# schusto/k-means-demo

Hardware: AMD Instinct MI355X
Metric: Lloyd iterations/sec (and point-assignments/sec) at N=1e8, D=128, K=1024, 1/2/4/8 MI355X (higher is better)
Workload: dtype bf16; 1 GPU; model=kmeans-lloyd N=1e8 D=128 K=1024, global_batch=100000000, seq_len=128, n_points=100000000, n_features=128, n_clusters=1024, parallelism=dp1

## Files before the change

### mikmeans/csrc/assign16.hip

```cpp
#include <cstdlib>
#include <type_traits>

#include "common.h"
#include "kernels.h"
#include "plan.h"
#include "tile.h"

namespace mk {

using plan::chunk_tiles16;

template <typename T, int DPAD, int P_, int CT_ = 0, int NBUF_ = 2, int NW_ = 4>
struct Assign16Cfg {
  static constexpr int NW = NW_;
  static constexpr int P = P_;
  static constexpr int V = Elem<T>::V;
  static constexpr int NQ = DPAD / 4 / V;
  static constexpr int TILE_BYTES = NQ * 1024;
  static constexpr int CT = CT_ ? CT_ : chunk_tiles16(sizeof(T), DPAD);
  static constexpr int CHUNK_BYTES = CT * TILE_BYTES;
  static constexpr int PIECES = CHUNK_BYTES / 1024;
  static constexpr int NPW = PIECES / NW;
  static constexpr int PTS = NW * P * 16;
  static constexpr int PP = (P + 3) / 4 * 4;
// ... 618 lines not shown
      blds16(rC, (MK_LDS void*)(dst + pc * 1024), loff, src + (uint32_t)pc * 1024u);
    }
  };
  const int64_t N = a.N;
  float* red = (float*)(bufs + C::NBUF * C::CHUNK_BYTES);
  float* opt = (float*)(bufs + C::NBUF * C::CHUNK_BYTES + 16 * C::NW);
  double* wacc = (double*)(bufs + C::NBUF * C::CHUNK_BYTES + 16 * C::NW + C::OPT_BYTES);
  uint32_t* xg_lds = (uint32_t*)(opt + C::NW * 16 * C::PP);
  uint32_t* el_lds = (uint32_t*)(bufs + C::NBUF * C::CHUNK_BYTES + 16 * C::NW + C::OPT_BYTES + 16 * C::NW);
  const unsigned kmask = key6_mask();
  const int G = (int)gridDim.x;
  int grp = (int)blockIdx.x;
  unsigned* ctr = g_persist_ctr[cslot];
  int* nxt_lds = (int*)(red + 2 * C::NW);
  int s0 = 0;

  const uint32_t rowb = (uint32_t)a.ldx * (uint32_t)sizeof(T);
  auto rows_of = [&](int gi) -> int {
    const int64_t left = N - (int64_t)gi * C::PTS;
    return left < C::PTS ? (int)left : C::PTS;
  };
  auto fresh_tid = []() -> int {
    int t = (int)threadIdx.x;
    asm volatile("" : "+v"(t));
    return t;
  };
  auto sx = [](int ln, int v, int o) -> int { return __builtin_amdgcn_ds_bpermute((ln ^ o) << 2, v); };
  auto sxf = [&](int ln, float v, int o) -> float { return __int_as_float(sx(ln, __float_as_int(v), o)); };
  auto lrow_of = [&](int tid, int p) -> int { return wid * (C::P * 16) + p * 16 + (tid & 15); };

// ... 30 lines not shown
  };

  if (a.timeline && threadIdx.x == 0) {
    const unsigned long long t = __builtin_amdgcn_s_memrealtime();
    a.timeline[(int64_t)grp * 8] = t;
    a.timeline[(int64_t)grp * 8 + 7] = t;
  }
  auto issue_cn = [&]() {
    const __amdgpu_buffer_rsrc_t rN = make_rsrc(a.cn, (uint32_t)a.Kpad * 4u);
    for (int pc = wid; pc < cn_bytes / 1024; pc += C::NW)
      blds16(rN, (MK_LDS void*)(cn_lds + pc * 1024), loff, (uint32_t)pc * 1024u);
  };
  issue_cn();
  issue_chunk(0, 0);
  load_group(grp);
  for (;;) {
    const int nvc = rows_of(grp);
    int nxt = 0;
    bool has_next = false;
    wait_vmcnt<0>();
    if (a.timeline && threadIdx.x == 0) a.timeline[(int64_t)grp * 8 + 6] = __builtin_amdgcn_s_memrealtime();
    float exn[EJ];
    exn[0] = __uint_as_float(xg_lds[fresh_tid()]);
    float off = 0.f;
    bool ppo = false;
    unsigned fetched;
    {
      const int ttid = fresh_tid();
      fetched = 0u;
      const int tln = ttid & 63, tr = ttid & 15, tg = tln >> 4;
      float m = 0.f, mn = 3.0e38f;
#pragma unroll
      for (int j = 0; j < EJ; ++j) { m = fmaxf(m, exn[j]); mn = fminf(mn, exn[j]); }
      m = fmaxf(m, sxf(tln, m, 16));
      mn = fminf(mn, sxf(tln, mn, 16));
      m = fmaxf(m, sxf(tln, m, 32));
      mn = fminf(mn, sxf(tln, mn, 32));
#pragma unroll
      for (int o = 1; o < 16; o <<= 1) {
        m = fmaxf(m, sxf(tln, m, o));
        mn = fminf(mn, sxf(tln, mn, o));
      }
      if (tln == 0) { red[2 * wid] = m; red[2 * wid + 1] = mn; }
      wait_lgkm0();
      raw_barrier();
      float mnw = 3.0e38f;
#pragma unroll
      for (int w = 0; w < C::NW; ++w) { off = fmaxf(off, red[2 * w]); mnw = fminf(mnw, red[2 * w + 1]); }
      ppo = __builtin_amdgcn_readfirstlane((int)(off > 4.f * mnw)) != 0;
      if (ttid == 0) fetched = atomicAdd(ctr, 1u);
      if (!ppo) {
        off = __builtin_fmaf(off, 2.44140625e-04f, off);
        off = __uint_as_float(__builtin_amdgcn_readfirstlane(__float_as_uint(off)));
        for (int kk = ttid; kk < a.Kpad; kk += C::NW * 64) ((float*)cn_lds)[kk] += off;
      } else {
        off = 0.f;
#pragma unroll
        for (int j = 0; j < EJ; ++j)
          if (4 * j + tg < C::P) opt[(wid * 16 + tr) * C::PP + 4 * j + tg] = __builtin_fmaf(exn[j], 2.44140625e-04f, exn[j]);
      }
    }

    float best[C::P], seg_best[C::P];
    int bg[C::P];
#pragma unroll
    for (int p = 0; p < C::P; ++p) { best[p] = 3.0e38f; seg_best[p] = 3.0e38f; bg[p] = 0; }

    auto chunk_head = [&](int c, auto last_tag) -> const char* {
      wait_vmcnt<0>();
      if constexpr (decltype(last_tag)::value) {
        if (fresh_tid() == 0) *nxt_lds = G + (int)fetched;
      }
      wait_lgkm0();
      raw_barrier();
      if constexpr (!decltype(last_tag)::value) {
        issue_chunk(c + 1, (s0 + c + 1) & 1);
      } else {
        nxt = __builtin_amdgcn_readfirstlane(*nxt_lds);
        has_next = nxt < ngroups;
        if (has_next) issue_chunk(0, (s0 + c + 1) & 1);
        const int tid = fresh_tid();
        const __amdgpu_buffer_rsrc_t rLo = make_rsrc(a.labels + (int64_t)grp * C::PTS, (uint32_t)nvc * 4u);
        blds4(rLo, (MK_LDS void*)(el_lds + wid * 64), (uint32_t)min(lrow_of(tid, (tid & 63) >> 4), nvc - 1) * 4u);
      }
      return bufs + ((s0 + c) & 1) * C::CHUNK_BYTES;
    };
    auto run_tile = [&](int c, int tl_i, const char* buf, auto ppo_tag, auto final_tag) {
      constexpr int PPO = decltype(ppo_tag)::value;
      constexpr bool FINAL = decltype(final_tag)::value;
      const int tile = c * C::CT + tl_i;
      u32x4 aw[C::NQ];
      const f32x4 ci = *(const f32x4*)(cn_lds + (tile * 16 + 4 * g) * 4);
      const char* tl = buf + tl_i * C::TILE_BYTES + lane * 16;
#pragma unroll
      for (int q = 0; q < C::NQ; ++q) aw[q] = *(const u32x4*)(tl + q * 1024);
// ... 127 lines not shown
      const unsigned long long t = __builtin_amdgcn_s_memrealtime();
      a.timeline[(int64_t)grp * 8 + 3] = t;
      if (has_next) {
        a.timeline[(int64_t)nxt * 8] = t;
        a.timeline[(int64_t)nxt * 8 + 7] = t;
      }
    }
    wait_lgkm0();
    raw_barrier();
    if (has_next) issue_cn();
    if (a.slots) {
      if (threadIdx.x == 0) {
        double si = 0, sc = 0;
#pragma unroll
        for (int w = 0; w < C::NW; ++w) { si += wacc[2 * w]; sc += wacc[2 * w + 1]; }
        slot_add((unsigned long long*)(a.slots + (grp % NSLOT) * SLOT_STRIDE), si, (long long)sc);
      }
    }
    if (!has_next) break;
    grp = nxt;
    s0 = (s0 + ncl) & 1;
  }
  wait_vmcnt<0>();
  if (threadIdx.x == 0 && atomicAdd(ctr + 1, 1u) == (unsigned)G - 1u) {
    atomicExch(ctr, 0u);
    atomicExch(ctr + 1, 0u);
  }
}

__global__ __launch_bounds__(256) void split_finish_kernel(AssignArgs a) {
  const int64_t i = (int64_t)blockIdx.x * 256 + threadIdx.x;
  float inert = 0.f;
  int changed = 0;
  if (i < a.N) {
    const unsigned long long key = a.split_keys[i];
    a.split_keys[i] = ~0ull;
    const int k = (int)(unsigned)key;
// ... 117 lines not shown
    if (cus[dev] < 1) return hipErrorInvalidValue;
  }
  int64_t grid = (int64_t)occ_blocks * cus[dev];
  if (cap > 0 && cap < grid) grid = cap;
  if (nblk < grid) grid = nblk;
  static int cslot = 0;
  cslot = (cslot + 1) % PERSIST_CTR_SLOTS;
  hipLaunchKernelGGL((assign16_persist_kernel<DPAD, P, OCC, PMAJ>), dim3((unsigned)grid), dim3(256), lds, s, b,
                     (int)nblk, cslot);
  return hipGetLastError();
}

constexpr size_t PERSIST_LDS_EXTRA = 1024;
constexpr int PERSIST_KPAD = 1024;
constexpr int64_t PERSIST_MIN_GROUPS = 196608;

template <typename T, int DPAD, int P, int CT_ = 0, int NBUF_ = 2, int OCC = 1, int NW_ = 4>
static hipError_t launch16_t(const AssignArgs& a, hipStream_t s) {
  using C = Assign16Cfg<T, DPAD, P, CT_, NBUF_, NW_>;
  if (a.Kpad % (16 * C::CT) != 0) return hipErrorInvalidValue;
  const int cn_bytes = ((a.Kpad * 4 + 1023) / 1024) * 1024;
  const size_t lds = cn_bytes + C::NBUF * C::CHUNK_BYTES + 16 * C::NW + C::OPT_BYTES + 16 * C::NW;
  if (lds > 160 * 1024) return hipErrorInvalidValue;
  const int64_t nblk = (a.N + C::PTS - 1) / C::PTS;
  if (nblk <= 0) return hipSuccess;
  const int splits = (a.split_keys && !a.ub && !a.n_dev) ? assign16_splits(nblk, a.Kpad / (16 * C::CT)) : 1;
  AssignArgs b = a;
  if ((a.ub != nullptr) != (a.lb != nullptr) || (a.scatter && !a.rows)) return hipErrorInvalidValue;
  if (splits == 1) b.split_keys = nullptr;
  const dim3 grid((unsigned)nblk, (unsigned)splits);
  if (g_timeline && nblk <= g_timeline_cap && splits == 1) b.timeline = g_timeline;
  b.epi_prefetch = variant(V_ASSIGN_EPI) != 0;
  b.early_prologue = variant(V_ASSIGN_EARLY) != 0;
  if constexpr (sizeof(T) == 2 && DPAD == 128 && P == 4 && CT_ == chunk_tiles16(2, 128) && NBUF_ == 2 && OCC == 4 &&
                NW_ == 4) {
    const int pv = variant(V_ASSIGN_PERSIST);
    const int pm = variant(V_ASSIGN_PMAJ);
    const bool applies = b.xn && !b.rows && !b.oseed && !b.split_keys && !b.n_dev && !b.ub && b.epi_prefetch &&
                         b.early_prologue && b.D == DPAD && (pm < 0 || pm == 1);
    const bool dflt = b.Kpad == PERSIST_KPAD && nblk >= PERSIST_MIN_GROUPS;
    if (applies && lds + PERSIST_LDS_EXTRA <= 160 * 1024 && (pv >= 0 ? pv != 0 : dflt))
      return launch16_persist<DPAD, P, OCC, 1>(b, nblk, lds + PERSIST_LDS_EXTRA, pv >= 2 ? pv : 0, s);
  }
  bool varg = false;
  constexpr bool VARG_OK = sizeof(T) == 2 && DPAD <= 64;
  if constexpr (VARG_OK) {
    const int e = variant(V_ASSIGN_VARG);
    varg = e >= 0 ? e != 0 : a.Kpad >= (DPAD == 64 ? 2048 : 1024);
  }
  if constexpr (VARG_OK) {
    if (varg) launch16_k<T, DPAD, P, CT_, NBUF_, OCC, NW_, true>(b, grid, lds, s);
    else launch16_k<T, DPAD, P, CT_, NBUF_, OCC, NW_, false>(b, grid, lds, s);
  } else {
    launch16_k<T, DPAD, P, CT_, NBUF_, OCC, NW_, false>(b, grid, lds, s);
  }
  if (splits > 1)
    hipLaunchKernelGGL(split_finish_kernel, dim3((unsigned)((a.N + 255) / 256)), dim3(256), 0, s, b);
// ... 52 lines not shown
int assign16_chunk_tiles(int dtype, int dpad) { return plan::assign16_chunk_tiles(dtype == DT_BF16 ? 2 : 4, dpad); }
int assign_kpad(int dtype, int dpad, int K) { return plan::assign_kpad(dtype == DT_BF16 ? 2 : 4, dpad, K); }
int assign_cn_len(int kpad) { return plan::assign_cn_len(kpad); }

int assign16_block_rows(int dtype, int dpad, int kpad) {
  int rows = 0;
  for_width(dtype, dpad, [&](auto t, auto w) {
    return assign_geometry<typename decltype(t)::type, decltype(w)::value>(kpad, false, [&](auto g) {
      rows = decltype(g)::ROWS;
      return 0;
    });
  });
  return rows;
}

hipError_t launch_assign16(int dtype, int dpad, const AssignArgs& a, hipStream_t s) {
  return (hipError_t)for_width(dtype, dpad, [&](auto t, auto w) {
    using T = typename decltype(t)::type;
    constexpr int DPAD = decltype(w)::value;
    return assign_geometry<T, DPAD>(a.Kpad, a.ub != nullptr, [&](auto g) {
      using G = decltype(g);
      return launch16_t<T, DPAD, G::P, G::CT, G::NBUF, G::OCC, G::NW>(a, s);
    });
  });
}

}
```

### mikmeans/csrc/binding.cpp

```cpp
#include <torch/extension.h>
#include <c10/hip/HIPStream.h>
#include <charconv>
#include <cmath>
#include <cstdlib>
#include <string>
#include <vector>

#include "jsnum.h"
#include "kernels.h"

namespace {

using at::Tensor;

void hip_check(hipError_t e, const char* what) {
  TORCH_CHECK(e == hipSuccess, "mikmeans: ", what, " failed: ", hipGetErrorString(e));
}
hipStream_t stream() { return c10::hip::getCurrentHIPStream().stream(); }

int dtype_of(const Tensor& X) {
  if (X.scalar_type() == at::kBFloat16) return mk::DT_BF16;
  TORCH_CHECK(X.scalar_type() == at::kFloat, "mikmeans: points must be bfloat16 or float32");
  return mk::DT_F32;
}
// ... 43 lines not shown
  TORCH_CHECK(pack.numel() >= rows * dpad, "mikmeans: pack too small (", pack.numel(), " < ", rows, " x ", dpad, ")");
  check_f32(cn, "cn", cn_min);
}
template <typename T>
T* opt_ptr(const c10::optional<Tensor>& t) {
  return t.has_value() && t->defined() ? reinterpret_cast<T*>(t->data_ptr()) : nullptr;
}

void check_i64(const Tensor& t, const char* name, int64_t numel_min);

void assign(const Tensor& X, const Tensor& pack, const Tensor& cn, const c10::optional<Tensor>& xn,
            const Tensor& labels, const c10::optional<Tensor>& mind,
            const c10::optional<Tensor>& slots, int64_t Kpad, int64_t dpad, bool track_changed,
            const c10::optional<Tensor>& keys, const c10::optional<Tensor>& rows,
            const c10::optional<Tensor>& ub, const c10::optional<Tensor>& lb, bool scatter,
            const c10::optional<Tensor>& count, const c10::optional<Tensor>& oseed) {
  const int dt = dtype_of(X);
  const int64_t ldx = check_points_dpad(X, dt, dpad);
  const bool gathered = rows.has_value() && rows->defined();
  if (gathered) {
    check_i64(*rows, "rows", 0);
    TORCH_CHECK(X.size(0) > 0 || rows->numel() == 0, "mikmeans: gathered rows from an empty X");
    TORCH_CHECK(!(keys.has_value() && keys->defined()), "mikmeans: gathered rows take the one-pass grid");
  }
  const int64_t N = gathered ? rows->numel() : X.size(0);
  TORCH_CHECK(!scatter || gathered, "mikmeans: scatter needs rows");
  const int64_t NO = scatter ? X.size(0) : N;
  const int D = (int)X.size(1);
  TORCH_CHECK(mk::assign_kpad(dt, (int)dpad, (int)Kpad) == Kpad, "mikmeans: bad Kpad ", Kpad, " for dpad ",
              dpad);
  const bool bounds = ub.has_value() && ub->defined();
// ... 29 lines not shown
  if (bounds) {
    a.ub = ub->data_ptr<float>();
    a.lb = lb->data_ptr<float>();
  }
  a.scatter = scatter ? 1 : 0;
  if (count.has_value() && count->defined()) {
    check_i64(*count, "count", 1);
    TORCH_CHECK(gathered && !(keys.has_value() && keys->defined()),
                "mikmeans: a device row count takes a gathered batch on the one-pass grid");
    a.n_dev = count->data_ptr<int64_t>();
  }
  if (oseed.has_value() && oseed->defined()) {
    TORCH_CHECK(dt == mk::DT_BF16, "mikmeans: seed offsets are the bf16 keys'");
    check_f32(*oseed, "oseed", X.size(0));
    a.oseed = oseed->data_ptr<float>();
  }
  hip_check(mk::launch_assign16(dt, (int)dpad, a, stream()), "assign");
}

void transform(const Tensor& X, const Tensor& pack, const Tensor& cn, int64_t K, int64_t Kpad, int64_t dpad,
               const Tensor& xn, const Tensor& out, bool squared) {
  const int dt = dtype_of(X);
  const int64_t ldx = check_points_dpad(X, dt, dpad);
  const int64_t N = X.size(0);
  TORCH_CHECK(mk::assign_kpad(dt, (int)dpad, (int)K) == Kpad, "mikmeans: bad Kpad ", Kpad);
  check_pack(pack, cn, X, Kpad, dpad, Kpad);
  check_f32(xn, "xn", N);
  check_cuda(out, "out");
  TORCH_CHECK(out.scalar_type() == at::kFloat && out.dim() == 2 && out.size(0) == N && out.size(1) == K &&
                  out.stride(1) == 1 && reinterpret_cast<uintptr_t>(out.data_ptr()) % 16 == 0,
// ... 638 lines not shown
  hip_check(e, "hipHostRegister");
  return true;
}
void host_unregister(const Tensor& t) {
  hip_check(hipHostUnregister(t.data_ptr()), "hipHostUnregister");
}

}

namespace mk {
static const char* const kVariantEnv[V_COUNT] = {"MIKMEANS_ASSIGN_VARG", "MIKMEANS_ASSIGN_PMAJ",
                                                 "MIKMEANS_ASSIGN_GEOM", "MIKMEANS_UPDATE_KS",
                                                 "MIKMEANS_UPDATE_KS_GM", "MIKMEANS_BLOBS_TPR",
                                                 "MIKMEANS_ASSIGN_TOP2_GEOM", "MIKMEANS_ASSIGN_EPI",
                                                 "MIKMEANS_ASSIGN_EARLY", "MIKMEANS_COLSTAT_BLOCKS",
                                                 "MIKMEANS_ASSIGN_PERSIST"};
static int* variant_table() {
  static int t[V_COUNT] = {};
  static const bool init = [] {
    for (int i = 0; i < V_COUNT; ++i) {
      const char* e = getenv(kVariantEnv[i]);
      t[i] = (e && *e) ? atoi(e) : -1;
    }
    return true;
  }();
  (void)init;
  return t;
}
int variant(Variant v) { return variant_table()[v]; }
void set_variant(Variant v, int value) { variant_table()[v] = value; }
}
// ... 43 lines not shown
  check_f32(ub, "ub", n);
  check_f32(lb, "lb", n);
  check_cuda(cand, "cand");
  TORCH_CHECK(cand.scalar_type() == at::kByte && cand.is_contiguous() && cand.numel() >= n,
              "mikmeans: cand must be contiguous uint8 [n]");
  check_f32(xn, "xn", n);
  check_f32(work, "work", 4);
  if (oseed.has_value()) check_f32(*oseed, "oseed", n);
  hip_check(mk::launch_tighten(dt, X.data_ptr(), ldx, (int)D, labels.data_ptr<int32_t>(), C.data_ptr<float>(),
                               C.stride(0), rows.data_ptr<int64_t>(), count.data_ptr<int64_t>(), rows.numel(),
                               ub.data_ptr<float>(), lb.data_ptr<float>(), cand.data_ptr<uint8_t>(),
                               xn.data_ptr<float>(), work.data_ptr<float>(), opt_ptr<const float>(oseed), stream()),
            "tighten");
}

void seed_offsets(const Tensor& xn, const Tensor& oseed, int64_t block_rows) {
  const int64_t n = xn.numel();
  check_f32(xn, "xn", n);
  check_f32(oseed, "oseed", n);
  TORCH_CHECK(block_rows > 0 && block_rows <= 4096, "mikmeans: bad block_rows ", block_rows);
  hip_check(mk::launch_seed_offsets(xn.data_ptr<float>(), n, (int)block_rows, oseed.data_ptr<float>(), stream()),
            "seed_offsets");
}

void bounds_update(const Tensor& labels, const Tensor& ub, const Tensor& lb, const Tensor& shift2, const Tensor& cn,
                   const Tensor& xn, const Tensor& cand, const Tensor& work, const c10::optional<Tensor>& oseed,
                   int64_t nterms) {
  const int64_t n = labels.numel();
  const int K = (int)shift2.numel();
  check_i32(labels, "labels", n);
// ... 53 lines not shown
  return s;
}

}

PYBIND11_MODULE(TORCH_EXTENSION_NAME, m) {
  m.doc() = "mikmeans native ops (gfx950 HIP kernels + host helpers)";
  m.def("kpar_select", &kpar_select, "k-means|| oversampling flags (philox keyed by the global row)");
  m.def("tighten", &tighten, "Hamerly tightening: exact distance to the label's centre for the candidates");
  m.def("compact", &compact, "rows of the nonzero flags, ascending; count on the device");
  m.def("compact_blocks", &mk::compact_blocks);
  m.def("assign", &assign, "fused MFMA distance + argmin (K2)", py::arg("X"), py::arg("pack"), py::arg("cn"),
        py::arg("xn"), py::arg("labels"), py::arg("mind"), py::arg("slots"), py::arg("Kpad"), py::arg("dpad"),
        py::arg("track_changed"), py::arg("keys") = py::none(), py::arg("rows") = py::none(),
        py::arg("ub") = py::none(), py::arg("lb") = py::none(), py::arg("scatter") = false,
        py::arg("count") = py::none(), py::arg("oseed") = py::none());
  m.def("seed_offsets", &seed_offsets, "the full assign's per-row bf16 seed offsets (bounded E-step)");
  m.def("assign_block_rows", [](int64_t dt, int64_t dpad, int64_t kpad) {
    return mk::assign16_block_rows((int)dt, (int)dpad, (int)kpad);
  }, "rows per workgroup of the full assign (its seed-offset block)");
  m.def("update", &update, "LDS-privatised per-cluster sums/counts (K3)", py::arg("X"), py::arg("labels"),
        py::arg("K"), py::arg("slab"), py::arg("cnt_slab"), py::arg("n_chunks"), py::arg("weights"),
        py::arg("col_exp"), py::arg("cnt_exp"), py::arg("clamp"), py::arg("clamp_count") = py::none(),
        py::arg("col_exp2") = py::none(), py::arg("rows") = py::none());
  m.def("transform", &transform, "distances of every row to every centre on the MFMA tiles", py::arg("X"),
        py::arg("pack"), py::arg("cn"), py::arg("K"), py::arg("Kpad"), py::arg("dpad"), py::arg("xn"), py::arg("out"),
        py::arg("squared") = false);
  m.def("topk", &topk, "the m nearest centres of every row (squared distances, ascending) on the MFMA tiles",
        py::arg("X"), py::arg("pack"), py::arg("cn"), py::arg("K"), py::arg("Kpad"), py::arg("dpad"), py::arg("xn"),
        py::arg("dist"), py::arg("idx"));
  m.def("partition", &partition,
// ... 136 lines not shown
```

### mikmeans/csrc/common.h

```cpp
#pragma once
#include <hip/hip_runtime.h>
#include <stdint.h>

namespace mk {

typedef short short8 __attribute__((ext_vector_type(8)));
typedef float f32x4 __attribute__((ext_vector_type(4)));
typedef float f32x16 __attribute__((ext_vector_type(16)));
typedef unsigned int u32x4 __attribute__((ext_vector_type(4)));

constexpr int WAVE = 64;
constexpr float PAD_SCORE = 1.0e30f;

#define MK_LDS __attribute__((address_space(3)))

__device__ __forceinline__ float bf16_to_f32(uint16_t h) {
  return __uint_as_float(((uint32_t)h) << 16);
}
__device__ __forceinline__ float bf16lo(uint32_t w) { return __uint_as_float(w << 16); }
__device__ __forceinline__ float bf16hi(uint32_t w) { return __uint_as_float(w & 0xffff0000u); }
__device__ __forceinline__ uint16_t f32_to_bf16(float f) {
  uint32_t u = __float_as_uint(f);
  if ((u & 0x7fffffffu) > 0x7f800000u) return (uint16_t)((u >> 16) | 0x40);
  u += 0x7fffu + ((u >> 16) & 1u);
// ... 143 lines not shown
  const unsigned long long bits = (unsigned long long)__double_as_longlong(v);
  const bool neg = bits >> 63;
  const int ex = (int)((bits >> 52) & 0x7ff);
  if (ex == 0x7ff) { atomicAdd(w + 6, SLOT_OVF); return; }
  unsigned long long m = (bits & ((1ull << 52) - 1)) | (ex ? (1ull << 52) : 0ull);
  int s = (ex ? ex : 1) - 1075 + 64;
  if (s < 0) { m = -s >= 64 ? 0ull : m >> -s; s = 0; }
  const int j0 = s >> 5, o = s & 31;
  if (j0 > 4) { atomicAdd(w + 6, SLOT_OVF); return; }
  const unsigned long long lo = m << o, hi = o ? (m >> (64 - o)) : 0ull;
  const unsigned long long d[3] = {lo & 0xffffffffull, lo >> 32, hi};
#pragma unroll
  for (int i = 0; i < 3; ++i)
    if (d[i]) atomicAdd(w + j0 + i, neg ? (unsigned long long)(-(long long)d[i]) : d[i]);
}
__device__ __forceinline__ double slot_decode(const long long* W) {
  if (W[6] >= (long long)(SLOT_OVF >> 1)) return __builtin_inf();
  double v = 0.0;
#pragma unroll
  for (int j = 6; j >= 0; --j) v += __builtin_ldexp((double)W[j], 32 * j - 64);
  return v;
}

__device__ __forceinline__ float pack_key(float s, int r) {
  return __uint_as_float((__float_as_uint(s) & ~15u) | (unsigned)r);
}
__device__ __forceinline__ float pack_key6(float s, unsigned mask, unsigned r) {
  return __uint_as_float((__float_as_uint(s) & mask) | r);
}
__device__ __forceinline__ unsigned key6_mask() {
// ... 31 lines not shown
```

### mikmeans/csrc/kernels.h

```cpp
#pragma once
#include <hip/hip_runtime.h>
#include <stdint.h>

#include "dispatch.h"
#include "fold.h"

namespace mk {

enum DType : int { DT_F32 = 0, DT_BF16 = 1 };
static_assert(DT_BF16 == WIDTH_BF16, "dispatch.h for_width takes these dtype codes");

constexpr int NSLOT = 256;
constexpr int SLOT_STRIDE = 8;

enum Variant { V_ASSIGN_VARG = 0, V_ASSIGN_PMAJ, V_ASSIGN_GEOM, V_UPDATE_KS, V_UPDATE_KS_GM, V_BLOBS_TPR,
               V_ASSIGN_TOP2_GEOM, V_ASSIGN_EPI, V_ASSIGN_EARLY, V_COLSTAT_BLOCKS, V_ASSIGN_PERSIST, V_COUNT };
int variant(Variant v);
void set_variant(Variant v, int value);

int assign16_chunk_tiles(int dtype, int dpad);
int assign_kpad(int dtype, int dpad, int K);
int assign_cn_len(int kpad);

struct AssignArgs {
  const void* X; int64_t N; int D; int64_t ldx;
  const void* Cpack; const float* cn; int Kpad;
  const float* xn;
  int32_t* labels;
  float* mind;
  double* slots;
  int track_changed;
  unsigned long long* split_keys = nullptr;
  const int64_t* rows = nullptr;
  float* ub = nullptr;
  float* lb = nullptr;
  int scatter = 0;
  const int64_t* n_dev = nullptr;
  const float* oseed = nullptr;
  unsigned long long* timeline = nullptr;
  int epi_prefetch = 1;
  int early_prologue = 1;
};
void set_assign_timeline(unsigned long long* buf, int64_t capacity);
hipError_t launch_assign16(int dtype, int dpad, const AssignArgs& a, hipStream_t s);
int assign16_block_rows(int dtype, int dpad, int kpad);
hipError_t launch_seed_offsets(const float* xn, int64_t n, int block_rows, float* oseed, hipStream_t s);

struct TransformArgs {
  const void* X; int64_t N; int D; int64_t ldx;
  const void* pack; const float* cn; int K; int Kpad;
  const float* xn;
  float* out; int64_t ldo;
  int squared;
};
hipError_t launch_transform(int dtype, int dpad, const TransformArgs& a, hipStream_t s);

constexpr int TOPK_MAX = 32;
struct TopkArgs {
  const void* X; int64_t N; int D; int64_t ldx;
  const void* pack; const float* cn; int K; int Kpad;
  const float* xn;
// ... 204 lines not shown
```

### mikmeans/csrc/rows.hip

```cpp
#include "common.h"
#include "kernels.h"

namespace mk {

constexpr uint32_t TAG_SMP = 0x53414D50u;

__device__ __forceinline__ int64_t sample_index(int64_t j, uint32_t step, uint32_t rank, int64_t n,
                                                uint32_t k0, uint32_t k1) {
  const U4 r = philox(U4{(uint32_t)j, step, rank, TAG_SMP}, k0, k1);
  const uint64_t w = ((uint64_t)r.y << 32) | r.x;
  const double u = (double)(w >> 11) * 0x1p-53;
  const int64_t i = (int64_t)(u * (double)n);
  return i < n ? i : n - 1;
}

template <typename T, int TPR>
__global__ __launch_bounds__(256) void sample_rows_kernel(const T* __restrict__ X, int64_t n, int64_t ldx,
                                                          int NP, T* __restrict__ out, int64_t ldo,
                                                          int64_t b, uint32_t k0, uint32_t k1,
                                                          uint32_t rank, uint32_t step, float* xn,
                                                          int64_t* idx_out) {
  constexpr int V = Elem<T>::V;
  const int64_t e = (int64_t)blockIdx.x * 256 + threadIdx.x;
  const int64_t j = e / TPR;
// ... 257 lines not shown
  const bool ppo = mx > 4.f * sn[0];
  const float off = __builtin_fmaf(mx, 2.44140625e-04f, mx);
  for (int64_t i = r0 + threadIdx.x; i < r1; i += 256)
    oseed[i] = ppo ? __builtin_fmaf(xn[i], 2.44140625e-04f, xn[i]) : off;
}

hipError_t launch_seed_offsets(const float* xn, int64_t n, int block_rows, float* oseed, hipStream_t s) {
  if (n <= 0) return hipSuccess;
  if (block_rows <= 0) return hipErrorInvalidValue;
  const int64_t nb = (n + block_rows - 1) / block_rows;
  if (nb > 0x7fffffff) return hipErrorInvalidValue;
  hipLaunchKernelGGL(seed_offsets_kernel, dim3((unsigned)nb), dim3(256), 0, s, xn, n, block_rows, oseed);
  return hipGetLastError();
}

hipError_t launch_bounds_update(const int32_t* labels, float* ub, float* lb, const float* shift2, const float* cn,
                                int K, const float* xn, int64_t n, uint8_t* cand, float* work, const float* oseed,
                                int nterms, hipStream_t s) {
  if (n <= 0) return hipSuccess;
  if (K < 1) return hipErrorInvalidValue;
  hipLaunchKernelGGL(shift_top2_kernel, dim3(1), dim3(1024), 0, s, shift2, cn, K, work);
  int64_t nb = (n + 255) / 256;
  if (nb > 8192) nb = 8192;
  hipLaunchKernelGGL(bounds_update_kernel, dim3((unsigned)nb), dim3(256), 0, s, labels, ub, lb, shift2, xn, n,
                     cand, work, oseed, nterms);
  return hipGetLastError();
}

template <typename T>
__global__ __launch_bounds__(256) void tighten_kernel(const T* __restrict__ X, int64_t ldx, int D,
// ... 193 lines not shown
```

### mikmeans/models/lloyd.py

```python
from __future__ import annotations

import contextlib
import math
import os
from dataclasses import dataclass, field

import torch

from ..ops import cpu as cpu_ops
from ..ops import native
from ..parallel.comm import Comm
from ..utils import profiling

_TRACE = os.environ.get("MIKMEANS_ROCTX", "0") not in ("", "0")


def _phase(name: str):
    return profiling.range(name) if _TRACE else contextlib.nullcontext()


@dataclass
class IterStats:
    iteration: int
    inertia: float
# ... 103 lines not shown
        self.stats = col_stats(self.X, xn=self.xn if fused else None)
        self.scales = mstep_scales(self.X, self.weights, comm=self.comm, stats=self.stats)
        if self.scales.nw and C.update_slice_width(self.dt, self.K, self.Dp, self.weights is not None) == 0:
            self.scales = MStepScales(self.scales.col_exp, self.scales.cnt_exp, [], dev)
        self.col_exp, self.cnt_exp = self.scales.col_exp, self.scales.cnt_exp
        if self.scales.nw:
            self.packed = torch.zeros(self.K * self.Dp + self.K + 2 + self.K * self.scales.nw,
                                      dtype=torch.float64, device=dev)
        if self.weights is not None or self.empty_policy == "farthest":
            self.mind = torch.empty(self.n, dtype=torch.float32, device=dev)
        if self.weights is not None:
            self._wscratch = torch.empty(C.WDOT_SCRATCH, dtype=torch.float64, device=dev)
        if self.bounded and self.segments > 1:
            native.warn_once("bounded E-step: not with segment overlap; full E-steps")
            self.bounded = False
        if self.bounded:
            self.ub = torch.empty(self.n, dtype=torch.float32, device=dev)
            self.lb = torch.empty(self.n, dtype=torch.float32, device=dev)
            self.cand = torch.empty(self.n, dtype=torch.uint8, device=dev)
            self._brows = torch.empty(self.n, dtype=torch.int64, device=dev)
            self._bcount = torch.zeros(1, dtype=torch.int64, device=dev)
            self._bscratch = torch.empty(max(1, C.compact_blocks(self.n)), dtype=torch.int64, device=dev)
            self._bwork = torch.empty(4, dtype=torch.float32, device=dev)
            self.qshift = torch.zeros(self.K, dtype=torch.float32, device=dev)
            self.oseed = self.pk.seed_offsets(self.xn) if self.n else None
            sxx = torch.zeros(1, dtype=torch.float64, device=dev)
            if self.n and self.weights is None:
                sxx += self.stats.sumsq[: self.Dp].to(device=dev, dtype=torch.float64).sum()
            elif self.n:
                C.wdot(self.xn, self.weights, sxx, self._wscratch)
# ... 19 lines not shown
                    self.delta = None

    def device_buffers(self) -> dict:
        from ..parallel.memplan import _r

        t = {"labels": self.labels, "xn": self.xn, "slab": self.slab, "cnt_slab": self.cnt_slab,
             "packed": self.packed, "C": self.C, "Cnew": self.Cnew, "shift": self.shift,
             "counts": self.counts, "pack": self.pk.pack, "cn": self.pk.cn, "slots": self.slots}
        if self.weights is not None:
            t["weights"] = self.weights
            t["wdot_scratch"] = self._wscratch
        if self.mind is not None:
            t["mind"] = self.mind
        if self.pk._keys is not None:
            t["split_keys"] = self.pk._keys
        if self.delta is not None:
            t.update(delta_prev=self.delta["prev"], delta_list=self.delta["list"],
                     delta_count=self.delta["count"], delta_tot=self.delta["tot"])
        if getattr(self, "bounded", False):
            t.update(bound_ub=self.ub, bound_lb=self.lb, bound_cand=self.cand, bound_rows=self._brows,
                     bound_count=self._bcount, bound_scratch=self._bscratch, bound_work=self._bwork,
                     bound_qshift=self.qshift)
            if self.oseed is not None:
                t["bound_oseed"] = self.oseed
        out = {k: _r(v.numel() * v.element_size()) for k, v in t.items()}
        for name in ("bufs", "stage"):
            bl = getattr(self, name, None)
            if bl:
                out["chunk_bufs" if name == "bufs" else "staging"] = sum(
                    _r(b.numel() * b.element_size()) for b in bl)
# ... 153 lines not shown

    def _pre_collective(self):
        C = self._C
        KD = self.K * self.Dp
        if self.n and self.segments > 1:
            self._assign_update_overlapped()
            C.reduce(self.slab, self.cnt_slab, self.n_chunks, self.K, self.Dp, self.slots, self.packed,
                     self.col_exp, self.cnt_exp)
            if self.weights is not None:
                self._weighted_inertia()
        elif self.n:
            with _phase("mikmeans.assign"):
                if self.bounded:
                    self._bounded_assign()
                else:
                    self.pk.assign(self.X, self.xn, self.labels, self.mind, self.slots, True)
            with _phase("mikmeans.update"):
                d = self.delta
                if d is not None:
                    if self.bounded:
                        C.label_delta_rows(self.labels, d["prev"], self._brows, self._bcount, d["list"], d["count"])
                    else:
                        C.label_delta(self.labels, d["prev"], d["list"], d["count"])
                    C.update_delta(self.X, self.labels, self.K, self.slab, self.cnt_slab, self.n_chunks,
                                   self.weights, self.col_exp, self.cnt_exp, d["list"], d["count"])
                    C.reduce_delta(self.slab, self.cnt_slab, self.n_chunks, self.K, self.Dp, self.slots,
                                   self.packed, self.col_exp, self.cnt_exp, d["tot"], d["count"],
                                   d["list"].shape[0])
                else:
                    C.update(self.X, self.labels, self.K, self.slab, self.cnt_slab, self.n_chunks,
                             self.weights, self.col_exp, self.cnt_exp, False)
# ... 208 lines not shown
```

### mikmeans/ops/__init__.py

```python
from __future__ import annotations

import torch

from . import cpu
from .native import available, dpad_for, dtype_code, require, vec_elems

__all__ = [
    "available",
    "require",
    "dpad_for",
    "vec_elems",
    "pad_columns",
    "pack_centers",
    "row_sqnorm",
    "assign",
    "cluster_sums",
    "CentroidPack",
]


def pad_columns(X: torch.Tensor, dtype: torch.dtype | None = None) -> torch.Tensor:
    dtype = dtype or X.dtype
    v = vec_elems(dtype)
    n, d = X.shape
# ... 34 lines not shown
        self.pack = torch.zeros(self.Kpad * self.dpad, dtype=dtype, device=device)
        self.cn = torch.zeros(C.assign_cn_len(self.Kpad), dtype=torch.float32, device=device)

    def load(self, centers: torch.Tensor) -> "CentroidPack":
        c = centers.to(device=self.pack.device, dtype=torch.float32).contiguous()
        assert c.shape == (self.K, self.D), (c.shape, self.K, self.D)
        self.finalize(0, None, c)
        return self

    def finalize(self, mode: int, packed, Cold, Cnew=None, frozen=None, mb_counts=None, shift=None,
                 counts=None, qshift=None):
        self._C.finalize(mode, packed, Cold, Cnew, frozen, mb_counts, self.pack, self.cn, shift, counts,
                         self.dpad, self.Kpad, qshift)

    def assign(self, X, xn, labels, mind=None, slots=None, track_changed: bool = False, rows=None,
               ub=None, lb=None, scatter: bool = False, count=None, oseed=None):
        if rows is not None:
            self._C.assign(X, self.pack, self.cn, xn, labels, mind, slots, self.Kpad, self.dpad,
                           track_changed, None, rows, ub, lb, scatter, count, oseed)
            return
        keys = None
        if 0 < X.shape[0] <= SPLIT_MAX_ROWS and ub is None:
            if self._keys is None or self._keys.numel() < X.shape[0]:
                self._keys = torch.full((X.shape[0],), -1, dtype=torch.int64, device=X.device)
            keys = self._keys
            if xn is not None and mind is None:
                mind = torch.empty(X.shape[0], dtype=torch.float32, device=X.device)
        self._C.assign(X, self.pack, self.cn, xn, labels, mind, slots, self.Kpad, self.dpad,
                       track_changed, keys, None, ub, lb, False, None, oseed)

    def seed_offsets(self, xn: torch.Tensor) -> "torch.Tensor | None":
        if self.dtype != torch.bfloat16:
            return None
        out = torch.empty(xn.numel(), dtype=torch.float32, device=xn.device)
        self._C.seed_offsets(xn, out, self._C.assign_block_rows(self.dt, self.dpad, self.Kpad))
        return out


def pack_centers(centers: torch.Tensor, D: int, dtype: torch.dtype, device):
    cen = torch.zeros((centers.shape[0], D), dtype=torch.float32, device=device)
    cen[:, : centers.shape[1]] = centers.to(device=device, dtype=torch.float32)
    return CentroidPack(cen.shape[0], D, dtype, device).load(cen)


# ... 296 lines not shown
```

### mikmeans/parallel/memplan.py

```python
from __future__ import annotations

import math
import os
from dataclasses import asdict, dataclass, field

HBM_BYTES = 288 * 10**9
GRANULE = 512
ROW_ALIGN = 1536
SPLIT_MAX_ROWS = 1 << 18
NSLOT, SLOT_STRIDE = 256, 8
WDOT_SCRATCH = 1024
COMPACT_ROWS = 4096
STAGING_BYTES = 1 << 26
UPD_LDS_MAX = 160 * 1024
KS_NT = 1024
KS_LIST_BYTES = 2 * (KS_NT // 64) * 64 * 4


class HBMCapacityError(MemoryError):
    """The requested fit cannot be placed in the GPU's HBM budget in any supported mode."""


def _r(nbytes: int) -> int:
    nbytes = int(nbytes)
# ... 213 lines not shown


def colstat_rows(es: int, n: int, Dp: int) -> int:
    V = 16 // es
    npt, rows = Dp // V, 0
    for p0 in range(0, npt, 64):
        L = 1
        while L < min(64, npt - p0):
            L *= 2
        rows = max(rows, min(colstat_cap(Dp), -(-n // (256 // L))))
    return rows


def _setup_items(n: int, Dp: int, es: int) -> dict:
    return {"colstat_part": _r(colstat_rows(es, n, Dp) * 3 * Dp * 8)} if n else {}


def plan_resident(n: int, D: int, K: int, dtype="bfloat16", *, weighted: bool = False,
                  incremental: bool = True, init="k-means++", n_local_trials: int | None = None,
                  copy_x: bool = True, empty_policy: str = "keep", bounded: bool = False,
                  src_itemsize: int | None = None) -> MemoryPlan:
    es = esize_of(dtype)
    Dp = padded_cols(D, es)
    wted = weighted
    p: dict = {}
    if copy_x:
        p["X"] = _r(n * Dp * es)
    if weighted:
        p["weights"] = _r(n * 4)
    p["labels"] = _r(n * 4)
    p["xn"] = _r(n * 4)
    if weighted or empty_policy == "farthest":
        p["mind"] = _r(n * 4)
    if weighted:
        p["wdot_scratch"] = _r(WDOT_SCRATCH * 8)
    nch = update_n_chunks(es, K, Dp, max(n, 1), wted or incremental)
    p["slab"] = _r(nch * K * Dp * 8)
    p["cnt_slab"] = _r(nch * K * 8)
    p["packed"] = _r((K * Dp + K + 2) * 8)
    p.update(_centroid_items(K, Dp, es))
    final = {"labels_out": _r(n * 4), "mind_out": _r(n * 4)}
    if 0 < n <= SPLIT_MAX_ROWS:
        if bounded:
            final["split_keys"] = _r(n * 8)
        else:
            p["split_keys"] = _r(n * 8)
    if incremental and n and n < 2**31 and choose_sw(es, K, Dp, True)[0] > 0:
        cap = max(1, min(n, int(n * 0.125)))
        p.update(delta_prev=_r(n * 4), delta_list=_r(cap * 8), delta_count=_r(4),
                 delta_tot=_r((K * Dp + K) * 8))
    if bounded:
        p.update(bound_ub=_r(n * 4), bound_lb=_r(n * 4), bound_cand=_r(n), bound_rows=_r(n * 8),
                 bound_count=_r(8), bound_scratch=_r(max(1, -(-n // COMPACT_ROWS)) * 8), bound_work=_r(16),
                 bound_qshift=_r(K * 4))
        if es == 2 and n:
# ... 165 lines not shown
```

Before: 44.05 iter/s.

## Precompute per-group xn max/min table and defer slot atomics in persistent assign

Adds a one-time kernel that computes each row group's max and min of xn and stores them in a table. The persistent bf16 assign kernel then reads this pair with a scalar load instead of doing a cross-wave shuffle reduction and a block barrier per group. It also vectorizes the centroid-norm offset add, and moves the slot atomics for each group into the next group's first chunk head so they overlap with loads. The cost is an extra table in HBM and more code paths.

```diff
diff --git a/mikmeans/csrc/assign16.hip b/mikmeans/csrc/assign16.hip
--- a/mikmeans/csrc/assign16.hip
+++ b/mikmeans/csrc/assign16.hip
@@ -656,6 +656,9 @@
   unsigned* ctr = g_persist_ctr[cslot];
   int* nxt_lds = (int*)(red + 2 * C::NW);
   int s0 = 0;
+  const bool gm = a.gmm != nullptr;
+  float gmx = 0.f, gmn = 0.f;
+  bool pend = false;
 
   const uint32_t rowb = (uint32_t)a.ldx * (uint32_t)sizeof(T);
   auto rows_of = [&](int gi) -> int {
@@ -716,6 +719,28 @@
   issue_cn();
   issue_chunk(0, 0);
   load_group(grp);
+  auto load_pair = [&](int gi) {
+    unsigned long long pr;
+    asm volatile("s_load_dwordx2 %0, %1, %2\n\ts_waitcnt lgkmcnt(0)"
+                 : "=&s"(pr) : "s"(a.gmm), "s"((unsigned)gi * 8u) : "memory");
+    gmx = __uint_as_float((unsigned)pr);
+    gmn = __uint_as_float((unsigned)(pr >> 32));
+  };
+  if (gm) load_pair(grp);
+  auto flush_slot = [&]() {
+    if (wid == 0 && fresh_tid() == 0) {
+      const unsigned* pk = (const unsigned*)red;
+      const unsigned pj0 = (unsigned)__builtin_amdgcn_readfirstlane((int)pk[3]), pcnt = pk[4];
+      const unsigned pg = (unsigned)__builtin_amdgcn_readfirstlane((int)pk[5]);
+      unsigned long long* w = (unsigned long long*)(a.slots + (pg % NSLOT) * SLOT_STRIDE);
+      if (pcnt) atomicAdd(w + 7, (unsigned long long)pcnt);
+      unsigned long long* wj = w + (pj0 & 7u);
+#pragma unroll
+      for (int i = 0; i < 3; ++i)
+        if (pk[i]) atomicAdd(wj + i, (pj0 & 8u) ? (unsigned long long)(-(long long)pk[i]) : (unsigned long long)pk[i]);
+    }
+    pend = false;
+  };
   for (;;) {
     const int nvc = rows_of(grp);
     int nxt = 0;
@@ -731,30 +756,45 @@
       const int ttid = fresh_tid();
       fetched = 0u;
       const int tln = ttid & 63, tr = ttid & 15, tg = tln >> 4;
-      float m = 0.f, mn = 3.0e38f;
-#pragma unroll
-      for (int j = 0; j < EJ; ++j) { m = fmaxf(m, exn[j]); mn = fminf(mn, exn[j]); }
-      m = fmaxf(m, sxf(tln, m, 16));
-      mn = fminf(mn, sxf(tln, mn, 16));
-      m = fmaxf(m, sxf(tln, m, 32));
-      mn = fminf(mn, sxf(tln, mn, 32));
-#pragma unroll
-      for (int o = 1; o < 16; o <<= 1) {
-        m = fmaxf(m, sxf(tln, m, o));
-        mn = fminf(mn, sxf(tln, mn, o));
-      }
-      if (tln == 0) { red[2 * wid] = m; red[2 * wid + 1] = mn; }
-      wait_lgkm0();
-      raw_barrier();
       float mnw = 3.0e38f;
-#pragma unroll
-      for (int w = 0; w < C::NW; ++w) { off = fmaxf(off, red[2 * w]); mnw = fminf(mnw, red[2 * w + 1]); }
+      if (gm) {
+        off = gmx;
+        mnw = gmn;
+      } else {
+        float m = 0.f, mn = 3.0e38f;
+#pragma unroll
+        for (int j = 0; j < EJ; ++j) { m = fmaxf(m, exn[j]); mn = fminf(mn, exn[j]); }
+        m = fmaxf(m, sxf(tln, m, 16));
+        mn = fminf(mn, sxf(tln, mn, 16));
+        m = fmaxf(m, sxf(tln, m, 32));
+        mn = fminf(mn, sxf(tln, mn, 32));
+#pragma unroll
+        for (int o = 1; o < 16; o <<= 1) {
+          m = fmaxf(m, sxf(tln, m, o));
+          mn = fminf(mn, sxf(tln, mn, o));
+        }
+        if (tln == 0) { red[2 * wid] = m; red[2 * wid + 1] = mn; }
+        wait_lgkm0();
+        raw_barrier();
+#pragma unroll
+        for (int w = 0; w < C::NW; ++w) { off = fmaxf(off, red[2 * w]); mnw = fminf(mnw, red[2 * w + 1]); }
+      }
       ppo = __builtin_amdgcn_readfirstlane((int)(off > 4.f * mnw)) != 0;
       if (ttid == 0) fetched = atomicAdd(ctr, 1u);
       if (!ppo) {
         off = __builtin_fmaf(off, 2.44140625e-04f, off);
         off = __uint_as_float(__builtin_amdgcn_readfirstlane(__float_as_uint(off)));
-        for (int kk = ttid; kk < a.Kpad; kk += C::NW * 64) ((float*)cn_lds)[kk] += off;
+        if (gm) {
+          for (int pc = wid; pc < cn_bytes / 1024; pc += C::NW) {
+            f32x4* cp = (f32x4*)(cn_lds + pc * 1024) + tln;
+            f32x4 cv = *cp;
+#pragma unroll
+            for (int j = 0; j < 4; ++j) cv[j] += off;
+            *cp = cv;
+          }
+        } else {
+          for (int kk = ttid; kk < a.Kpad; kk += C::NW * 64) ((float*)cn_lds)[kk] += off;
+        }
       } else {
         off = 0.f;
 #pragma unroll
@@ -775,12 +815,14 @@
       }
       wait_lgkm0();
       raw_barrier();
+      if (c == 0 && pend) flush_slot();
       if constexpr (!decltype(last_tag)::value) {
         issue_chunk(c + 1, (s0 + c + 1) & 1);
       } else {
         nxt = __builtin_amdgcn_readfirstlane(*nxt_lds);
         has_next = nxt < ngroups;
         if (has_next) issue_chunk(0, (s0 + c + 1) & 1);
+        if (gm) load_pair(has_next ? nxt : grp);
         const int tid = fresh_tid();
         const __amdgpu_buffer_rsrc_t rLo = make_rsrc(a.labels + (int64_t)grp * C::PTS, (uint32_t)nvc * 4u);
         blds4(rLo, (MK_LDS void*)(el_lds + wid * 64), (uint32_t)min(lrow_of(tid, (tid & 63) >> 4), nvc - 1) * 4u);
@@ -938,13 +980,28 @@
         double si = 0, sc = 0;
 #pragma unroll
         for (int w = 0; w < C::NW; ++w) { si += wacc[2 * w]; sc += wacc[2 * w + 1]; }
-        slot_add((unsigned long long*)(a.slots + (grp % NSLOT) * SLOT_STRIDE), si, (long long)sc);
-      }
+        const SlotDigits sd = slot_split(si);
+        unsigned long long* w = (unsigned long long*)(a.slots + (grp % NSLOT) * SLOT_STRIDE);
+        if (sd.ovf) atomicAdd(w + 6, SLOT_OVF);
+        if (!gm) {
+          if ((long long)sc) atomicAdd(w + 7, (unsigned long long)(long long)sc);
+#pragma unroll
+          for (int i = 0; i < 3; ++i)
+            if (sd.d[i])
+              atomicAdd(w + (sd.j0 & 7u) + i, (sd.j0 & 8u) ? (unsigned long long)(-(long long)sd.d[i]) : (unsigned long long)sd.d[i]);
+        } else {
+          unsigned* pk = (unsigned*)red;
+          pk[0] = sd.d[0]; pk[1] = sd.d[1]; pk[2] = sd.d[2]; pk[3] = sd.j0;
+          pk[4] = (unsigned)(int)sc; pk[5] = (unsigned)grp;
+        }
+      }
+      pend = gm;
     }
     if (!has_next) break;
     grp = nxt;
     s0 = (s0 + ncl) & 1;
   }
+  if (pend) flush_slot();
   wait_vmcnt<0>();
   if (threadIdx.x == 0 && atomicAdd(ctr + 1, 1u) == (unsigned)G - 1u) {
     atomicExch(ctr, 0u);
@@ -1092,6 +1149,7 @@
 constexpr size_t PERSIST_LDS_EXTRA = 1024;
 constexpr int PERSIST_KPAD = 1024;
 constexpr int64_t PERSIST_MIN_GROUPS = 196608;
+constexpr bool PERSIST_GMM_DEFAULT = true;
 
 template <typename T, int DPAD, int P, int CT_ = 0, int NBUF_ = 2, int OCC = 1, int NW_ = 4>
 static hipError_t launch16_t(const AssignArgs& a, hipStream_t s) {
@@ -1117,8 +1175,11 @@
     const bool applies = b.xn && !b.rows && !b.oseed && !b.split_keys && !b.n_dev && !b.ub && b.epi_prefetch &&
                          b.early_prologue && b.D == DPAD && (pm < 0 || pm == 1);
     const bool dflt = b.Kpad == PERSIST_KPAD && nblk >= PERSIST_MIN_GROUPS;
-    if (applies && lds + PERSIST_LDS_EXTRA <= 160 * 1024 && (pv >= 0 ? pv != 0 : dflt))
+    if (applies && lds + PERSIST_LDS_EXTRA <= 160 * 1024 && (pv >= 0 ? pv != 0 : dflt)) {
+      const int gv = variant(V_ASSIGN_GMM);
+      if (!(gv >= 0 ? gv != 0 : PERSIST_GMM_DEFAULT)) b.gmm = nullptr;
       return launch16_persist<DPAD, P, OCC, 1>(b, nblk, lds + PERSIST_LDS_EXTRA, pv >= 2 ? pv : 0, s);
+    }
   }
   bool varg = false;
   constexpr bool VARG_OK = sizeof(T) == 2 && DPAD <= 64;
@@ -1201,6 +1262,15 @@
   return rows;
 }
 
+bool assign16_uses_gmm(int dtype, int dpad, int kpad, int64_t n) {
+  if (dtype != DT_BF16 || dpad != 128 || n <= 0 || assign16_block_rows(dtype, dpad, kpad) != 256) return false;
+  const int pv = variant(V_ASSIGN_PERSIST), pm = variant(V_ASSIGN_PMAJ), gv = variant(V_ASSIGN_GMM);
+  if (variant(V_ASSIGN_EPI) == 0 || variant(V_ASSIGN_EARLY) == 0 || !(pm < 0 || pm == 1)) return false;
+  const bool dflt = kpad == PERSIST_KPAD && (n + 255) / 256 >= PERSIST_MIN_GROUPS;
+  if (!(pv >= 0 ? pv != 0 : dflt)) return false;
+  return gv >= 0 ? gv != 0 : PERSIST_GMM_DEFAULT;
+}
+
 hipError_t launch_assign16(int dtype, int dpad, const AssignArgs& a, hipStream_t s) {
   return (hipError_t)for_width(dtype, dpad, [&](auto t, auto w) {
     using T = typename decltype(t)::type;
diff --git a/mikmeans/csrc/binding.cpp b/mikmeans/csrc/binding.cpp
--- a/mikmeans/csrc/binding.cpp
+++ b/mikmeans/csrc/binding.cpp
@@ -81,7 +81,8 @@
             const c10::optional<Tensor>& slots, int64_t Kpad, int64_t dpad, bool track_changed,
             const c10::optional<Tensor>& keys, const c10::optional<Tensor>& rows,
             const c10::optional<Tensor>& ub, const c10::optional<Tensor>& lb, bool scatter,
-            const c10::optional<Tensor>& count, const c10::optional<Tensor>& oseed) {
+            const c10::optional<Tensor>& count, const c10::optional<Tensor>& oseed,
+            const c10::optional<Tensor>& gmm) {
   const int dt = dtype_of(X);
   const int64_t ldx = check_points_dpad(X, dt, dpad);
   const bool gathered = rows.has_value() && rows->defined();
@@ -141,6 +142,13 @@
     TORCH_CHECK(dt == mk::DT_BF16, "mikmeans: seed offsets are the bf16 keys'");
     check_f32(*oseed, "oseed", X.size(0));
     a.oseed = oseed->data_ptr<float>();
+  }
+  if (gmm.has_value() && gmm->defined()) {
+    TORCH_CHECK(dt == mk::DT_BF16 && !gathered && xn.has_value(), "mikmeans: the group table is the full bf16 pass's");
+    const int br = mk::assign16_block_rows(dt, (int)dpad, (int)Kpad);
+    TORCH_CHECK(br > 0, "mikmeans: no group size for this shape");
+    check_f32(*gmm, "gmm", 2 * ((N + br - 1) / br));
+    a.gmm = gmm->data_ptr<float>();
   }
   hip_check(mk::launch_assign16(dt, (int)dpad, a, stream()), "assign");
 }
@@ -809,7 +817,7 @@
                                                  "MIKMEANS_UPDATE_KS_GM", "MIKMEANS_BLOBS_TPR",
                                                  "MIKMEANS_ASSIGN_TOP2_GEOM", "MIKMEANS_ASSIGN_EPI",
                                                  "MIKMEANS_ASSIGN_EARLY", "MIKMEANS_COLSTAT_BLOCKS",
-                                                 "MIKMEANS_ASSIGN_PERSIST"};
+                                                 "MIKMEANS_ASSIGN_PERSIST", "MIKMEANS_ASSIGN_GMM"};
 static int* variant_table() {
   static int t[V_COUNT] = {};
   static const bool init = [] {
@@ -883,6 +891,15 @@
             "tighten");
 }
 
+void group_minmax(const Tensor& xn, const Tensor& out, int64_t block_rows) {
+  const int64_t n = xn.numel();
+  check_f32(xn, "xn", n);
+  TORCH_CHECK(block_rows > 0 && block_rows <= 4096, "mikmeans: bad block_rows ", block_rows);
+  check_f32(out, "gmm", 2 * ((n + block_rows - 1) / block_rows));
+  hip_check(mk::launch_group_minmax(xn.data_ptr<float>(), n, (int)block_rows, out.data_ptr<float>(), stream()),
+            "group_minmax");
+}
+
 void seed_offsets(const Tensor& xn, const Tensor& oseed, int64_t block_rows) {
   const int64_t n = xn.numel();
   check_f32(xn, "xn", n);
@@ -966,7 +983,11 @@
         py::arg("xn"), py::arg("labels"), py::arg("mind"), py::arg("slots"), py::arg("Kpad"), py::arg("dpad"),
         py::arg("track_changed"), py::arg("keys") = py::none(), py::arg("rows") = py::none(),
         py::arg("ub") = py::none(), py::arg("lb") = py::none(), py::arg("scatter") = false,
-        py::arg("count") = py::none(), py::arg("oseed") = py::none());
+        py::arg("count") = py::none(), py::arg("oseed") = py::none(), py::arg("gmm") = py::none());
+  m.def("group_minmax", &group_minmax, "{max, min} of xn per row group (the persistent assign's table)");
+  m.def("assign_uses_gmm", [](int64_t dt, int64_t dpad, int64_t kpad, int64_t n) {
+    return mk::assign16_uses_gmm((int)dt, (int)dpad, (int)kpad, n);
+  }, "whether a plain full assign of this shape reads the per-group table");
   m.def("seed_offsets", &seed_offsets, "the full assign's per-row bf16 seed offsets (bounded E-step)");
   m.def("assign_block_rows", [](int64_t dt, int64_t dpad, int64_t kpad) {
     return mk::assign16_block_rows((int)dt, (int)dpad, (int)kpad);
diff --git a/mikmeans/csrc/common.h b/mikmeans/csrc/common.h
--- a/mikmeans/csrc/common.h
+++ b/mikmeans/csrc/common.h
@@ -181,6 +181,26 @@
   for (int i = 0; i < 3; ++i)
     if (d[i]) atomicAdd(w + j0 + i, neg ? (unsigned long long)(-(long long)d[i]) : d[i]);
 }
+struct SlotDigits { unsigned d[3]; unsigned j0; bool ovf; };
+__device__ __forceinline__ SlotDigits slot_split(double v) {
+  SlotDigits r = {{0u, 0u, 0u}, 0u, false};
+  if (v == 0.0) return r;
+  const unsigned long long bits = (unsigned long long)__double_as_longlong(v);
+  const bool neg = bits >> 63;
+  const int ex = (int)((bits >> 52) & 0x7ff);
+  if (ex == 0x7ff) { r.ovf = true; return r; }
+  unsigned long long m = (bits & ((1ull << 52) - 1)) | (ex ? (1ull << 52) : 0ull);
+  int s = (ex ? ex : 1) - 1075 + 64;
+  if (s < 0) { m = -s >= 64 ? 0ull : m >> -s; s = 0; }
+  const int j0 = s >> 5, o = s & 31;
+  if (j0 > 4) { r.ovf = true; return r; }
+  const unsigned long long lo = m << o, hi = o ? (m >> (64 - o)) : 0ull;
+  r.d[0] = (unsigned)(lo & 0xffffffffull);
+  r.d[1] = (unsigned)(lo >> 32);
+  r.d[2] = (unsigned)hi;
+  r.j0 = (unsigned)j0 | (neg ? 8u : 0u);
+  return r;
+}
 __device__ __forceinline__ double slot_decode(const long long* W) {
   if (W[6] >= (long long)(SLOT_OVF >> 1)) return __builtin_inf();
   double v = 0.0;
diff --git a/mikmeans/csrc/kernels.h b/mikmeans/csrc/kernels.h
--- a/mikmeans/csrc/kernels.h
+++ b/mikmeans/csrc/kernels.h
@@ -14,7 +14,8 @@
 constexpr int SLOT_STRIDE = 8;
 
 enum Variant { V_ASSIGN_VARG = 0, V_ASSIGN_PMAJ, V_ASSIGN_GEOM, V_UPDATE_KS, V_UPDATE_KS_GM, V_BLOBS_TPR,
-               V_ASSIGN_TOP2_GEOM, V_ASSIGN_EPI, V_ASSIGN_EARLY, V_COLSTAT_BLOCKS, V_ASSIGN_PERSIST, V_COUNT };
+               V_ASSIGN_TOP2_GEOM, V_ASSIGN_EPI, V_ASSIGN_EARLY, V_COLSTAT_BLOCKS, V_ASSIGN_PERSIST, V_ASSIGN_GMM,
+               V_COUNT };
 int variant(Variant v);
 void set_variant(Variant v, int value);
 
@@ -37,6 +38,7 @@
   int scatter = 0;
   const int64_t* n_dev = nullptr;
   const float* oseed = nullptr;
+  const float* gmm = nullptr;
   unsigned long long* timeline = nullptr;
   int epi_prefetch = 1;
   int early_prologue = 1;
@@ -45,6 +47,8 @@
 hipError_t launch_assign16(int dtype, int dpad, const AssignArgs& a, hipStream_t s);
 int assign16_block_rows(int dtype, int dpad, int kpad);
 hipError_t launch_seed_offsets(const float* xn, int64_t n, int block_rows, float* oseed, hipStream_t s);
+hipError_t launch_group_minmax(const float* xn, int64_t n, int block_rows, float* out, hipStream_t s);
+bool assign16_uses_gmm(int dtype, int dpad, int kpad, int64_t n);
 
 struct TransformArgs {
   const void* X; int64_t N; int D; int64_t ldx;
diff --git a/mikmeans/csrc/rows.hip b/mikmeans/csrc/rows.hip
--- a/mikmeans/csrc/rows.hip
+++ b/mikmeans/csrc/rows.hip
@@ -295,6 +295,40 @@
   return hipGetLastError();
 }
 
+__global__ __launch_bounds__(256) void group_minmax_kernel(const float* __restrict__ xn, int64_t n, int block_rows,
+                                                          int64_t nb, float* __restrict__ out) {
+  const int lane = threadIdx.x & 63;
+  const int64_t gidx = (int64_t)blockIdx.x * 4 + (threadIdx.x >> 6);
+  if (gidx >= nb) return;
+  const int64_t r0 = gidx * block_rows;
+  const int64_t r1 = r0 + block_rows < n ? r0 + block_rows : n;
+  float m = 0.f, mn = 3.0e38f;
+  for (int64_t i = r0 + lane; i < r1; i += 64) {
+    const float v = xn[i];
+    m = fmaxf(m, v);
+    mn = fminf(mn, v);
+  }
+#pragma unroll
+  for (int o = 32; o > 0; o >>= 1) {
+    m = fmaxf(m, __shfl_xor(m, o, 64));
+    mn = fminf(mn, __shfl_xor(mn, o, 64));
+  }
+  if (lane == 0) {
+    out[2 * gidx] = m;
+    out[2 * gidx + 1] = mn;
+  }
+}
+
+hipError_t launch_group_minmax(const float* xn, int64_t n, int block_rows, float* out, hipStream_t s) {
+  if (n <= 0) return hipSuccess;
+  if (block_rows <= 0) return hipErrorInvalidValue;
+  const int64_t nb = (n + block_rows - 1) / block_rows;
+  const int64_t grid = (nb + 3) / 4;
+  if (grid > 0x7fffffff) return hipErrorInvalidValue;
+  hipLaunchKernelGGL(group_minmax_kernel, dim3((unsigned)grid), dim3(256), 0, s, xn, n, block_rows, nb, out);
+  return hipGetLastError();
+}
+
 hipError_t launch_bounds_update(const int32_t* labels, float* ub, float* lb, const float* shift2, const float* cn,
                                 int K, const float* xn, int64_t n, uint8_t* cand, float* work, const float* oseed,
                                 int nterms, hipStream_t s) {
diff --git a/mikmeans/models/lloyd.py b/mikmeans/models/lloyd.py
--- a/mikmeans/models/lloyd.py
+++ b/mikmeans/models/lloyd.py
@@ -141,6 +141,11 @@
         if self.bounded and self.segments > 1:
             native.warn_once("bounded E-step: not with segment overlap; full E-steps")
             self.bounded = False
+        self.gmm = None
+        from ..ops import SPLIT_MAX_ROWS
+        if (self.n > SPLIT_MAX_ROWS and not self.bounded and self.segments == 1
+                and self.pk.uses_group_minmax(self.n)):
+            self.gmm = self.pk.group_minmax(self.xn)
         if self.bounded:
             self.ub = torch.empty(self.n, dtype=torch.float32, device=dev)
             self.lb = torch.empty(self.n, dtype=torch.float32, device=dev)
@@ -190,6 +195,8 @@
             t["mind"] = self.mind
         if self.pk._keys is not None:
             t["split_keys"] = self.pk._keys
+        if getattr(self, "gmm", None) is not None:
+            t["group_minmax"] = self.gmm
         if self.delta is not None:
             t.update(delta_prev=self.delta["prev"], delta_list=self.delta["list"],
                      delta_count=self.delta["count"], delta_tot=self.delta["tot"])
@@ -373,7 +380,7 @@
                 if self.bounded:
                     self._bounded_assign()
                 else:
-                    self.pk.assign(self.X, self.xn, self.labels, self.mind, self.slots, True)
+                    self.pk.assign(self.X, self.xn, self.labels, self.mind, self.slots, True, gmm=self.gmm)
             with _phase("mikmeans.update"):
                 d = self.delta
                 if d is not None:
diff --git a/mikmeans/ops/__init__.py b/mikmeans/ops/__init__.py
--- a/mikmeans/ops/__init__.py
+++ b/mikmeans/ops/__init__.py
@@ -72,7 +72,7 @@
                          self.dpad, self.Kpad, qshift)
 
     def assign(self, X, xn, labels, mind=None, slots=None, track_changed: bool = False, rows=None,
-               ub=None, lb=None, scatter: bool = False, count=None, oseed=None):
+               ub=None, lb=None, scatter: bool = False, count=None, oseed=None, gmm=None):
         if rows is not None:
             self._C.assign(X, self.pack, self.cn, xn, labels, mind, slots, self.Kpad, self.dpad,
                            track_changed, None, rows, ub, lb, scatter, count, oseed)
@@ -85,7 +85,16 @@
             if xn is not None and mind is None:
                 mind = torch.empty(X.shape[0], dtype=torch.float32, device=X.device)
         self._C.assign(X, self.pack, self.cn, xn, labels, mind, slots, self.Kpad, self.dpad,
-                       track_changed, keys, None, ub, lb, False, None, oseed)
+                       track_changed, keys, None, ub, lb, False, None, oseed, gmm)
+
+    def uses_group_minmax(self, n: int) -> bool:
+        return bool(self._C.assign_uses_gmm(self.dt, self.dpad, self.Kpad, int(n)))
+
+    def group_minmax(self, xn: torch.Tensor) -> torch.Tensor:
+        br = self._C.assign_block_rows(self.dt, self.dpad, self.Kpad)
+        out = torch.empty((-(-xn.numel() // br), 2), dtype=torch.float32, device=xn.device)
+        self._C.group_minmax(xn, out, br)
+        return out
 
     def seed_offsets(self, xn: torch.Tensor) -> "torch.Tensor | None":
         if self.dtype != torch.bfloat16:
diff --git a/mikmeans/parallel/memplan.py b/mikmeans/parallel/memplan.py
--- a/mikmeans/parallel/memplan.py
+++ b/mikmeans/parallel/memplan.py
@@ -251,6 +251,18 @@
 
 def _setup_items(n: int, Dp: int, es: int) -> dict:
     return {"colstat_part": _r(colstat_rows(es, n, Dp) * 3 * Dp * 8)} if n else {}
+
+
+PERSIST_DPAD, PERSIST_KPAD, PERSIST_GROUP_ROWS, PERSIST_MIN_GROUPS = 128, 1024, 256, 196608
+PERSIST_GMM_DEFAULT = True
+
+
+def group_minmax_bytes(n: int, Dp: int, K: int, es: int, bounded: bool = False) -> int:
+    dpad = dpad_for(Dp, es)
+    groups = _cdiv(n, PERSIST_GROUP_ROWS)
+    on = (PERSIST_GMM_DEFAULT and es == 2 and dpad == PERSIST_DPAD and not bounded
+          and assign_kpad(es, dpad, K) == PERSIST_KPAD and groups >= PERSIST_MIN_GROUPS)
+    return _r(groups * 8) if on else 0
 
 
 def plan_resident(n: int, D: int, K: int, dtype="bfloat16", *, weighted: bool = False,
@@ -276,6 +288,8 @@
     p["cnt_slab"] = _r(nch * K * 8)
     p["packed"] = _r((K * Dp + K + 2) * 8)
     p.update(_centroid_items(K, Dp, es))
+    if group_minmax_bytes(n, Dp, K, es, bounded):
+        p["group_minmax"] = group_minmax_bytes(n, Dp, K, es, bounded)
     final = {"labels_out": _r(n * 4), "mind_out": _r(n * 4)}
     if 0 < n <= SPLIT_MAX_ROWS:
         if bounded:
```

Measured after the change: 44.41 iter/s, median of 6. Within noise of the previous version (+0.8%).
